# lfalive/fast-genomic-data-processing

Hardware: AMD Instinct MI355X
Metric: PairHMM GCUPS (higher is better)
Workload: dtype f32

## Files before the change

fast-genomic-data-processing_amd/csrc/pairhmm_kernels.hip.inc:

```

#include <type_traits>

namespace {

struct Job {
    uint64_t read_off;
    uint64_t hap_off;
    uint32_t R;
    uint32_t H;
    uint32_t pair;
    uint32_t pad_;
};
static_assert(sizeof(Job) == 32, "Job is 32 bytes");

struct KernelArgs {
    const Job* jobs;
    const uint32_t* job_list;
    const uint32_t* n_dyn;
    uint32_t n_static;
    uint32_t job_first;
    const uint8_t* bases;
    const uint8_t* qual;
    const uint8_t* ins;
    const uint8_t* del;
    const uint8_t* gcp;
    const uint8_t* hap_bases;
    const void* ph2pr;
    const void* mm;
    const void* ph2pr_div3;
    const void* gap_ratio;
    double* out_log10;
    uint8_t* used_f64;
    uint32_t* rerun_list;
    uint32_t* rerun_count;
    uint32_t lds_stride;
    void* strip_scratch;
    uint32_t strip_stride;
    float log10_initial_f;
    double log10_initial_d;
};

constexpr double kExactBelow = 1e-280;
constexpr int kCodeN = 4;
constexpr int kCodePad = 7;

__device__ __forceinline__ int base_code(int b) {
    int c = 0;
    c = (b == 'C') ? 1 : c;
    c = (b == 'T') ? 2 : c;
    c = (b == 'G') ? 3 : c;
    c = (b == 'N') ? kCodeN : c;
    return c;
}

__device__ __forceinline__ uint32_t base_code4(uint32_t w) {
    const uint32_t sel = (w >> 1) & 0x07070707u;
    const uint32_t code = __builtin_amdgcn_perm(0x04000000u, 0x03020100u, sel);
    const uint32_t want = __builtin_amdgcn_perm(0x4E000000u, 0x47544341u, sel);
    const uint32_t diff = want ^ w;
    const uint32_t nz = (((diff & 0x7F7F7F7Fu) + 0x7F7F7F7Fu) | diff) & 0x80808080u;
    const uint32_t ok = ((nz ^ 0x80808080u) >> 7) * 0xFFu;
    return code & ok;
}

template <int G> constexpr int lane_stride() { return G < 16 ? 16 / G : 1; }

template <int G>
__device__ __forceinline__ int dpp_shr1(int old, int v) {
    if constexpr (G == 64)
        return __builtin_amdgcn_update_dpp(old, v, 0x138 , 0xf, 0xf, false);
    else
        return __builtin_amdgcn_update_dpp(old, v, 0x110 + lane_stride<G>() , 0xf, 0xf, false);
}
template <int G>
__device__ __forceinline__ float shr1(float old, float v) {
    return __builtin_bit_cast(float, dpp_shr1<G>(__builtin_bit_cast(int, old), __builtin_bit_cast(int, v)));
}
template <int G>
__device__ __forceinline__ double shr1(double old, double v) {
    long long o = __builtin_bit_cast(long long, old), x = __builtin_bit_cast(long long, v);
    unsigned lo = (unsigned)dpp_shr1<G>((int)(unsigned)o, (int)(unsigned)x);
    unsigned hi = (unsigned)dpp_shr1<G>((int)(unsigned)(o >> 32), (int)(unsigned)(x >> 32));
    return __builtin_bit_cast(double, ((long long)hi << 32) | (long long)lo);
}

template <int G, typename T>
__device__ __forceinline__ T shr1_down(T v) {
    const int lane = (int)(threadIdx.x & 63);
    constexpr int S = lane_stride<G>();
    const int j = G < 16 ? (lane & 15) / S : lane % G;
    const int src = (j == G - 1) ? lane : lane + S;
    return __shfl(v, src, 64);
}

__device__ __forceinline__ float fma_(float a, float b, float c) { return __builtin_fmaf(a, b, c); }
__device__ __forceinline__ double fma_(double a, double b, double c) { return __builtin_fma(a, b, c); }

template <typename T> struct Prec;
template <> struct Prec<float> {
    static __device__ __forceinline__ float initial() { return 0x1p120f; }
};
template <> struct Prec<double> {
    static __device__ __forceinline__ double initial() { return 0x1p1020; }
};

#ifndef MGX_PAIRHMM_CODES
#define MGX_PAIRHMM_CODES 5
#endif
constexpr int kNumCodes = MGX_PAIRHMM_CODES;
template <int RPL> constexpr int etab_bytes_per_wave() { return ((RPL + 1) / 2) * kNumCodes * 64 * 8; }

template <typename T, int G, int RPL, bool STRIP = false, bool EXACT = false>
__device__ __forceinline__ void pairhmm_body(const KernelArgs& a, uint8_t* smem, const uint32_t block, const uint32_t n_blocks) {
    constexpr int GPW = 64 / G;
    constexpr bool kETab = (sizeof(T) == 4);
    constexpr int RP2 = (RPL + 1) / 2;
    constexpr int S = lane_stride<G>();
    const int gpb = (int)blockDim.x / G;
    const int tid = (int)threadIdx.x;
    const int lane = tid & 63;
    const int wave = tid >> 6;
    const int j = G < 16 ? (lane & 15) / S : lane % G;
    const int grp = wave * GPW + (G < 16 ? (lane >> 4) * S + (lane & 15) % S : lane / G);
    const int n_waves = (int)blockDim.x >> 6;
    uint8_t* etab = smem + (kETab ? (size_t)wave * etab_bytes_per_wave<RPL>() : 0);
    uint8_t* hapbuf = smem + (kETab ? (size_t)n_waves * etab_bytes_per_wave<RPL>() : 0) +
                      (size_t)grp * a.lds_stride;
    const T* __restrict__ ph2pr = (const T*)a.ph2pr;
    const T* __restrict__ mm = (const T*)a.mm;
    const T* __restrict__ ph2pr_div3 = (const T*)a.ph2pr_div3;
    const T* __restrict__ gap_ratio = (const T*)a.gap_ratio;
    const uint32_t n_jobs = a.n_dyn ? *a.n_dyn : a.n_static;

    for (uint32_t base = block * (uint32_t)gpb; base < n_jobs; base += n_blocks * (uint32_t)gpb) {
        const uint32_t slot = base + (uint32_t)grp;
        const bool live = slot < n_jobs;
        uint32_t job_idx = 0;
        Job job;
        job.read_off = 0; job.hap_off = 0; job.R = 0; job.H = 0; job.pair = 0; job.pad_ = 0;
        if (live) {
            job_idx = a.job_list ? a.job_list[slot] : a.job_first + slot;
            job = a.jobs[job_idx];
        }
        const int R = (int)job.R, H = (int)job.H;
        constexpr int kStripRows = G * RPL;
        const int n_strips = STRIP ? (R > kStripRows ? (R + kStripRows - 1) / kStripRows : 1) : 1;
        const int first_rows = R - (n_strips - 1) * kStripRows;

        __syncthreads();
        bool hap_n = false;
        {
            const uint8_t* hp = a.hap_bases + job.hap_off;
            const int n_words = (int)a.lds_stride >> 2;
            uint32_t* hb32 = reinterpret_cast<uint32_t*>(hapbuf);
            for (int w = j; w < n_words; w += G) {
                const int c0 = 4 * w - G;
                uint32_t packed;
                if (live && c0 >= 0 && c0 + 4 <= H) {
                    uint32_t raw;
                    __builtin_memcpy(&raw, hp + c0, 4);
                    packed = base_code4(raw);
                } else {
                    packed = 0;
#pragma unroll
                    for (int t = 0; t < 4; ++t) {
                        const int c = c0 + t;
                        const int code = (live && c >= 0 && c < H) ? base_code(hp[c]) : (kNumCodes > 4 ? kCodeN : 0);
                        packed |= (uint32_t)code << (8 * t);
                    }
                }
                if constexpr (kETab && kNumCodes == 4) {
                    const uint32_t x = packed ^ (0x01010101u * (uint32_t)kCodeN);
                    hap_n |= ((x - 0x01010101u) & ~x & 0x80808080u) != 0;
                    packed &= 0x03030303u;
                }
                hb32[w] = packed;
            }
        }
        bool group_hap_n = false;
        if constexpr (kETab && kNumCodes == 4) {
            uint64_t gmask;
            if constexpr (G == 64) gmask = ~0ull;
            else if constexpr (G == 16) gmask = 0xFFFFull << (lane & 48);
            else gmask = (uint64_t)((G == 8 ? 0x5555u : 0x1111u) << ((lane & 15) % S)) << (lane & 48);
            group_hap_n = (__ballot((int)hap_n) & gmask) != 0;
        }

        T sumM = 0, sumX = 0;
        bool zero_gap = false;
        if constexpr (STRIP) {
            for (int rr = lane; rr < R; rr += 64) zero_gap |= (a.gcp[job.read_off + (uint64_t)rr] & 127) == 0;
        }
        int nl = 0;
        T* const bnd = STRIP ? reinterpret_cast<T*>(a.strip_scratch) + (size_t)block * 6u * a.strip_stride : nullptr;
      for (int strip = 0; strip < n_strips; ++strip) {
        const int rows_here = (STRIP && strip > 0) ? kStripRows : first_rows;
        const int row_base = (STRIP && strip > 0) ? first_rows + (strip - 1) * kStripRows : 0;
        const bool last_strip = strip == n_strips - 1;
        nl = (rows_here + RPL - 1) / RPL;
        const int top_clones = nl * RPL - rows_here;
        volatile T* const bcur = STRIP ? bnd + (size_t)(strip & 1) * 3u * a.strip_stride : nullptr;
        const volatile T* const bprev = STRIP ? bnd + (size_t)((strip & 1) ^ 1) * 3u * a.strip_stride : nullptr;
        if (STRIP && strip > 0) __syncthreads();

        T k0[RPL], k1[RPL], k2[RPL], k3[RPL], k4[RPL], eM[RPL], eX[RPL];
        int rb[RPL];
        T pm[RPL], px[RPL], py[RPL];
        bool clone[RPL];
        T ratio[RPL];
        const T init_y = Prec<T>::initial() / (T)(H > 0 ? H : 1);
#pragma unroll
        for (int s = 0; s < RPL; ++s) {
            const int rho = j * RPL + s - top_clones;
            k0[s] = 0; k1[s] = 0; k2[s] = 0; k3[s] = 0; k4[s] = 0; eM[s] = 0; eX[s] = 0;
            rb[s] = 0; pm[s] = 0; px[s] = 0; py[s] = 0; clone[s] = false; ratio[s] = 0;
            if (live && j < nl) {
                if (rho < 0) {
                    clone[s] = true;
                    k3[s] = 1;
                    py[s] = init_y;
                } else {
                    const uint64_t o = job.read_off + (uint64_t)(row_base + rho);
                    const int qi = a.ins[o] & 127, qd = a.del[o] & 127, qc = a.gcp[o] & 127;
                    const int qq = a.qual[o] & 127;
                    const int mn = qi <= qd ? qi : qd, mx = qi <= qd ? qd : qi;
                    k0[s] = mm[((mx * (mx + 1)) >> 1) + mn];
                    k3[s] = ph2pr[qc];
                    k1[s] = (T)1.0 - ph2pr[qc];
                    k2[s] = ph2pr[qi];
                    k4[s] = ph2pr[qd];
                    zero_gap |= (qc == 0);
                    const T distm = ph2pr[qq];
                    eM[s] = (T)1.0 - distm;
                    const int code = base_code(a.bases[o]);
                    eX[s] = (code == kCodeN) ? eM[s] : ph2pr_div3[qq];
                    ratio[s] = gap_ratio[qc];
                    rb[s] = code;
                }
            }
        }
        if constexpr (kETab) {
            float* et = reinterpret_cast<float*>(etab) + lane * 2;
#pragma unroll
            for (int s = 0; s < RPL; ++s)
#pragma unroll
                for (int code = 0; code < kNumCodes; ++code)
                    et[((s >> 1) * kNumCodes + code) * 128 + (s & 1)] =
                        (code == rb[s] || code == kCodeN) ? eM[s] : eX[s];
        }
        __syncthreads();

        const int nsteps_g = live ? (H + nl - 1) : 0;
        int nmax = nsteps_g, nmin = live ? nsteps_g : 0x7fffffff;
        if constexpr (GPW > 1) {
#pragma unroll
            for (int off = 1; off < 64; off <<= 1) {
                if (off >= S && off < (G < 16 ? 16 : G)) continue;
                const int o1 = __shfl_xor(nmax, off, 64), o2 = __shfl_xor(nmin, off, 64);
                nmax = o1 > nmax ? o1 : nmax;
                nmin = o2 < nmin ? o2 : nmin;
            }
        }
        nmax = __builtin_amdgcn_readfirstlane(nmax);
        nmin = __builtin_amdgcn_readfirstlane(nmin);
        if (nmin > nmax) nmin = nmax;

        const uint8_t* hp_lane = hapbuf + (G - j);
        const uint8_t* et_lane = etab + lane * 8;

        auto load_e = [&](int h, T (&dst)[RPL]) {
            if constexpr (kETab) {
                const uint8_t* p = et_lane + (h << 9);
#pragma unroll
                for (int s2 = 0; s2 < RP2; ++s2) {
                    const float2 v = *reinterpret_cast<const float2*>(p + s2 * kNumCodes * 512);
                    dst[2 * s2] = v.x;
                    if (2 * s2 + 1 < RPL) dst[2 * s2 + 1] = v.y;
                }
            } else {
                const bool hN = (h == kCodeN);
#pragma unroll
                for (int s = 0; s < RPL; ++s) dst[s] = ((h == rb[s]) | hN) ? eM[s] : eX[s];
            }
        };

        const bool use_plain = EXACT || __any((int)zero_gap) != 0;

        auto sweep = [&](auto scaled_tag) {
            constexpr bool SC = decltype(scaled_tag)::value;
            T y_above = init_y;
            if constexpr (SC) {
                T g_own[RPL], g_below[RPL];
#pragma unroll
                for (int s = 0; s < RPL; ++s) g_own[s] = k1[s];
                T g_next_lane = shr1_down<G>(g_own[0]);
#pragma unroll
                for (int s = 0; s < RPL; ++s) g_below[s] = (s + 1 < RPL) ? g_own[s + 1] : g_next_lane;
                if (j == nl - 1) {
                    g_below[RPL - 1] = (T)1.0;
                    if constexpr (STRIP) { if (!last_strip) g_below[RPL - 1] = (T)1.0 - ph2pr[a.gcp[job.read_off + (uint64_t)(row_base + rows_here)] & 127]; }
                }
#pragma unroll
                for (int s = 0; s < RPL; ++s) {
                    if (clone[s]) {
                        py[s] = g_below[s] * init_y;
                    } else {
                        const T gb = g_below[s];
                        const T pMX = k2[s], pXX = k3[s], pMY = k4[s];
                        k1[s] = gb * pMX;
                        k2[s] = gb * ratio[s];
                        k3[s] = gb * pMY;
                        k4[s] = pXX;
                    }
                    if (clone[s]) { k1[s] = 0; k2[s] = 0; k3[s] = 0; k4[s] = 1; }
                }
                y_above = g_own[0] * init_y;
            }
            const T old_y = (j == 0) ? y_above : (T)0;
            T uaM = 0, uaX = 0, uaY = old_y, ubM = 0, ubX = 0, ubY = old_y;
            if constexpr (STRIP) {
                if (strip > 0) {
                    uaY = 0; ubY = 0;
                    if (j == 0 && H > 0) { ubM = bprev[0]; ubX = bprev[a.strip_stride]; ubY = bprev[2u * a.strip_stride]; }
                }
            }

            auto column = [&](const T (&ec)[RPL], T& o2M, T& o2X, T& o2Y, const T o1M, const T o1X, bool count, const int dcol) {
                T Mn[RPL], Xn[RPL], Yn[RPL];
                if constexpr (SC) {
                    Mn[0] = (fma_(o2M, k0[0], o2X) + o2Y) * ec[0];
                    Xn[0] = fma_(o1X, k2[0], o1M * k1[0]);
                    Yn[0] = fma_(py[0], k4[0], pm[0] * k3[0]);
#pragma unroll
                    for (int s = 1; s < RPL; ++s) {
                        Mn[s] = (fma_(pm[s - 1], k0[s], px[s - 1]) + py[s - 1]) * ec[s];
                        Xn[s] = fma_(Xn[s - 1], k2[s], Mn[s - 1] * k1[s]);
                        Yn[s] = fma_(py[s], k4[s], pm[s] * k3[s]);
                    }
                } else if constexpr (EXACT) {
                    Mn[0] = ((o2M * k0[0] + o2X * k1[0]) + o2Y * k1[0]) * ec[0];
                    Xn[0] = o1M * k2[0] + o1X * k3[0];
                    Yn[0] = pm[0] * k4[0] + py[0] * k3[0];
#pragma unroll
                    for (int s = 1; s < RPL; ++s) {
                        Mn[s] = ((pm[s - 1] * k0[s] + px[s - 1] * k1[s]) + py[s - 1] * k1[s]) * ec[s];
                        Xn[s] = Mn[s - 1] * k2[s] + Xn[s - 1] * k3[s];
                        Yn[s] = pm[s] * k4[s] + py[s] * k3[s];
                    }
                } else {
                    Mn[0] = fma_(o2Y, k1[0], fma_(o2X, k1[0], o2M * k0[0])) * ec[0];
                    Xn[0] = fma_(o1X, k3[0], o1M * k2[0]);
                    Yn[0] = fma_(py[0], k3[0], pm[0] * k4[0]);
#pragma unroll
                    for (int s = 1; s < RPL; ++s) {
                        Mn[s] = fma_(py[s - 1], k1[s], fma_(px[s - 1], k1[s], pm[s - 1] * k0[s])) * ec[s];
                        Xn[s] = fma_(Xn[s - 1], k3[s], Mn[s - 1] * k2[s]);
                        Yn[s] = fma_(py[s], k3[s], pm[s] * k4[s]);
                    }
                }
#pragma unroll
                for (int s = 0; s < RPL; ++s) { pm[s] = Mn[s]; px[s] = Xn[s]; py[s] = Yn[s]; }
                if (count && (!STRIP || last_strip)) { sumM += Mn[RPL - 1]; sumX += Xn[RPL - 1]; }
                o2M = shr1<G>(o2M, Mn[RPL - 1]);
                o2X = shr1<G>(o2X, Xn[RPL - 1]);
                o2Y = shr1<G>(o2Y, Yn[RPL - 1]);
                if constexpr (STRIP) {
                    if (strip > 0 && j == 0) {
                        const int c1 = dcol + 1;
                        const bool in = c1 < H;
                        o2M = in ? bprev[c1] : (T)0; o2X = in ? bprev[a.strip_stride + c1] : (T)0; o2Y = in ? bprev[2u * a.strip_stride + c1] : (T)0;
                    }
                    if (!last_strip && j == nl - 1) {
                        const int c = dcol - j;
                        if (c >= 0 && c < H) { bcur[c] = Mn[RPL - 1]; bcur[a.strip_stride + c] = Xn[RPL - 1]; bcur[2u * a.strip_stride + c] = Yn[RPL - 1]; }
                    }
                }
            };

            T e[RPL];
            int d = 0;
            int h1 = hp_lane[1];
            load_e((int)hp_lane[0], e);
            for (; d + 2 <= nmin; d += 2) {
                T e1[RPL];
                load_e(h1, e1);
                const int h2 = hp_lane[d + 2], h3 = hp_lane[d + 3];
                column(e, uaM, uaX, uaY, ubM, ubX, true, d);
                load_e(h2, e);
                column(e1, ubM, ubX, ubY, uaM, uaX, true, d + 1);
                h1 = h3;
            }
            for (; d < nmax; ++d) {
                const int hn = hp_lane[d + 1];
                column(e, uaM, uaX, uaY, ubM, ubX, d < nsteps_g, d);
                T t;
                t = uaM; uaM = ubM; ubM = t;
                t = uaX; uaX = ubX; ubX = t;
                t = uaY; uaY = ubY; ubY = t;
                load_e(hn, e);
            }
        };
        if constexpr (EXACT) sweep(std::integral_constant<bool, false>{});
        else if (use_plain) sweep(std::integral_constant<bool, false>{});
        else sweep(std::integral_constant<bool, true>{});
      }

        if (live && j == nl - 1) {
            const T res = sumM + sumX;
            if constexpr (sizeof(T) == 4) {
                if (res < 1e-28f || group_hap_n) {
                    const uint32_t k = atomicAdd(a.rerun_count, 1u);
                    a.rerun_list[k] = job_idx;
                } else {
                    a.out_log10[job.pair] = (double)(log10f(res) - a.log10_initial_f);
                }
            } else {
                if (!EXACT && a.rerun_count && res < kExactBelow) {
                    const uint32_t k = atomicAdd(a.rerun_count, 1u);
                    a.rerun_list[k] = job_idx;
                } else {
                    a.out_log10[job.pair] = log10(res) - a.log10_initial_d;
                    a.used_f64[job.pair] = 1;
                }
            }
        }
    }
}

typedef float f2 __attribute__((ext_vector_type(2)));
__device__ __forceinline__ f2 pk_fma(f2 a, f2 b, f2 c) { return __builtin_elementwise_fma(a, b, c); }

constexpr int kPkCodes = 4;
constexpr int kPkRowStride = kPkCodes * 64 * 4 + 4;
template <int P> constexpr int etab_pk_bytes_per_wave() { return (2 * P * kPkRowStride + 15) & ~15; }

template <int G, int P>
__device__ __forceinline__ void pairhmm_body_pk(const KernelArgs& a, uint8_t* smem, const uint32_t block, const uint32_t n_blocks) {
    typedef float T;
    constexpr int RPL = 2 * P;
    constexpr int GPW = 64 / G;
    constexpr int S = lane_stride<G>();
    constexpr int PAD = 2 * G;
    const int gpb = (int)blockDim.x / G;
    const int tid = (int)threadIdx.x;
    const int lane = tid & 63;
    const int wave = tid >> 6;
    const int j = G < 16 ? (lane & 15) / S : lane % G;
    const int grp = wave * GPW + (G < 16 ? (lane >> 4) * S + (lane & 15) % S : lane / G);
    const int n_waves = (int)blockDim.x >> 6;
    uint8_t* etab = smem + (size_t)wave * etab_pk_bytes_per_wave<P>();
    uint8_t* hapbuf = smem + (size_t)n_waves * etab_pk_bytes_per_wave<P>() + (size_t)grp * a.lds_stride;
    const T* __restrict__ ph2pr = (const T*)a.ph2pr;
    const T* __restrict__ mm = (const T*)a.mm;
    const T* __restrict__ ph2pr_div3 = (const T*)a.ph2pr_div3;
    const T* __restrict__ gap_ratio = (const T*)a.gap_ratio;
    const uint32_t n_jobs = a.n_dyn ? *a.n_dyn : a.n_static;

    for (uint32_t base = block * (uint32_t)gpb; base < n_jobs; base += n_blocks * (uint32_t)gpb) {
        const uint32_t slot = base + (uint32_t)grp;
        const bool live = slot < n_jobs;
        uint32_t job_idx = 0;
        Job job;
        job.read_off = 0; job.hap_off = 0; job.R = 0; job.H = 0; job.pair = 0; job.pad_ = 0;
        if (live) {
            job_idx = a.job_list ? a.job_list[slot] : a.job_first + slot;
            job = a.jobs[job_idx];
        }
        const int R = (int)job.R, H = (int)job.H;

        __syncthreads();
        bool to_f64 = false;
        {
            const uint8_t* hp = a.hap_bases + job.hap_off;
            const int n_words = (int)a.lds_stride >> 2;
            uint32_t* hb32 = reinterpret_cast<uint32_t*>(hapbuf);
            for (int w = j; w < n_words; w += G) {
                const int c0 = 4 * w - PAD;
                uint32_t packed;
                if (live && c0 >= 0 && c0 + 4 <= H) {
                    uint32_t raw;
                    __builtin_memcpy(&raw, hp + c0, 4);
                    packed = base_code4(raw);
                } else {
                    packed = 0;
#pragma unroll
                    for (int t = 0; t < 4; ++t) {
                        const int c = c0 + t;
                        const int code = (live && c >= 0 && c < H) ? base_code(hp[c]) : 0;
                        packed |= (uint32_t)code << (8 * t);
                    }
                }
                const uint32_t x = packed ^ (0x01010101u * (uint32_t)kCodeN);
                to_f64 |= ((x - 0x01010101u) & ~x & 0x80808080u) != 0;
                hb32[w] = packed & 0x03030303u;
            }
        }

        const int nh = (R + P - 1) / P;
        const int top_clones = nh * P - R;
        const int qf = nh - 1;
        const T init_y = Prec<T>::initial() / (T)(H > 0 ? H : 1);

        T g_own[RPL];
#pragma unroll
        for (int t = 0; t < RPL; ++t) {
            const int rho = j * RPL + t - top_clones;
            const int q = 2 * j + (t >= P ? 1 : 0);
            g_own[t] = 0;
            if (live && q < nh && rho >= 0) {
                const int qc = a.gcp[job.read_off + (uint64_t)rho] & 127;
                g_own[t] = (T)1.0 - ph2pr[qc];
                to_f64 |= (qc == 0);
            }
        }
        const T g_next_lane = shr1_down<G>(g_own[0]);
        f2 K0[P], K1[P], K2[P], K3[P], K4[P], pm[P], px[P], py[P];
        {
            float* et = reinterpret_cast<float*>(etab) + lane;
#pragma unroll
            for (int t = 0; t < RPL; ++t) {
                const int rho = j * RPL + t - top_clones;
                const int q = 2 * j + (t >= P ? 1 : 0);
                T gb = (t + 1 < RPL) ? g_own[t + 1] : g_next_lane;
                if (j == (qf >> 1) && t == ((qf & 1) ? RPL - 1 : P - 1)) gb = (T)1.0;
                T c0 = 0, cA = 0, cB = 0, cC = 0, cD = 0, y0 = 0, eM = 0, eX = 0;
                int rb = 0;
                if (live && q < nh) {
                    if (rho < 0) {
                        cD = 1; y0 = gb * init_y;
                    } else {
                        const uint64_t o = job.read_off + (uint64_t)rho;
                        const int qi = a.ins[o] & 127, qd = a.del[o] & 127, qc = a.gcp[o] & 127;
                        const int qq = a.qual[o] & 127;
                        const int mn = qi <= qd ? qi : qd, mx = qi <= qd ? qd : qi;
                        c0 = mm[((mx * (mx + 1)) >> 1) + mn];
                        cA = gb * ph2pr[qi];
                        cB = gb * gap_ratio[qc];
                        cC = gb * ph2pr[qd];
                        cD = ph2pr[qc];
                        eM = (T)1.0 - ph2pr[qq];
                        rb = base_code(a.bases[o]);
                        eX = (rb == kCodeN) ? eM : ph2pr_div3[qq];
                    }
                }
#pragma unroll
                for (int code = 0; code < kPkCodes; ++code)
                    et[t * (kPkRowStride / 4) + code * 64] = (code == rb) ? eM : eX;
                const int k = t % P;
                if (t < P) { K0[k].x = c0; K1[k].x = cA; K2[k].x = cB; K3[k].x = cC; K4[k].x = cD; py[k].x = y0; }
                else       { K0[k].y = c0; K1[k].y = cA; K2[k].y = cB; K3[k].y = cC; K4[k].y = cD; py[k].y = y0; }
            }
        }
#pragma unroll
        for (int k = 0; k < P; ++k) { pm[k] = f2{0, 0}; px[k] = f2{0, 0}; }
        const T y_above = g_own[0] * init_y;
        const T py_mid = py[P - 1].x;
        __syncthreads();

        const int nsteps_g = live ? (H + nh - 1) : 0;
        int nmax = nsteps_g, nmin = live ? nsteps_g : 0x7fffffff;
        if constexpr (GPW > 1) {
#pragma unroll
            for (int off = 1; off < 64; off <<= 1) {
                if (off >= S && off < (G < 16 ? 16 : G)) continue;
                const int o1 = __shfl_xor(nmax, off, 64), o2 = __shfl_xor(nmin, off, 64);
                nmax = o1 > nmax ? o1 : nmax;
                nmin = o2 < nmin ? o2 : nmin;
            }
        }
        nmax = __builtin_amdgcn_readfirstlane(nmax);
        nmin = __builtin_amdgcn_readfirstlane(nmin);
        if (nmin > nmax) nmin = nmax;

        const uint8_t* hp_lane = hapbuf + (PAD - 2 * j);
        const uint8_t* et_lane = etab + lane * 4;
        uint64_t gmask;
        if constexpr (G == 64) gmask = ~0ull;
        else if constexpr (G == 16) gmask = 0xFFFFull << (lane & 48);
        else gmask = (uint64_t)((G == 8 ? 0x5555u : 0x1111u) << ((lane & 15) % S)) << (lane & 48);
        const bool group_to_f64 = (__ballot((int)to_f64) & gmask) != 0;

        f2 sumM = {0, 0}, sumX = {0, 0};

        {
            const T old_y = (j == 0) ? y_above : (T)0;
            f2 uaM = {0, 0}, uaX = {0, 0}, uaY = {old_y, py_mid}, ubM = {0, 0}, ubX = {0, 0}, ubY = {old_y, py_mid};

            auto column = [&](const f2 (&ec)[P], f2& o2M, f2& o2X, f2& o2Y, const f2 o1M, const f2 o1X, bool count) {
                f2 Mn[P], Xn[P], Yn[P];
                Mn[0] = (pk_fma(o2M, K0[0], o2X) + o2Y) * ec[0];
                Xn[0] = pk_fma(o1X, K2[0], o1M * K1[0]);
                Yn[0] = pk_fma(py[0], K4[0], pm[0] * K3[0]);
#pragma unroll
                for (int k = 1; k < P; ++k) {
                    Mn[k] = (pk_fma(pm[k - 1], K0[k], px[k - 1]) + py[k - 1]) * ec[k];
                    Xn[k] = pk_fma(Xn[k - 1], K2[k], Mn[k - 1] * K1[k]);
                    Yn[k] = pk_fma(py[k], K4[k], pm[k] * K3[k]);
                }
#pragma unroll
                for (int k = 0; k < P; ++k) { pm[k] = Mn[k]; px[k] = Xn[k]; py[k] = Yn[k]; }
                if (count) { sumM += Mn[P - 1]; sumX += Xn[P - 1]; }
                o2M.x = shr1<G>(o2M.x, Mn[P - 1].y); o2M.y = Mn[P - 1].x;
                o2X.x = shr1<G>(o2X.x, Xn[P - 1].y); o2X.y = Xn[P - 1].x;
                o2Y.x = shr1<G>(o2Y.x, Yn[P - 1].y); o2Y.y = Yn[P - 1].x;
            };
            auto load_e = [&](int h, int hprev, f2 (&dst)[P]) {
                const uint8_t* pc = et_lane + (h << 8);
                const uint8_t* pp = et_lane + (hprev << 8) + P * kPkRowStride;
#pragma unroll
                for (int k = 0; k < P; ++k) {
                    dst[k].x = *reinterpret_cast<const float*>(pc + k * kPkRowStride);
                    dst[k].y = *reinterpret_cast<const float*>(pp + k * kPkRowStride);
                }
            };

            f2 e[P];
            int d = 0;
            int h0 = hp_lane[0], h1 = hp_lane[1];
            load_e(h0, (int)hp_lane[-1], e);
            for (; d + 2 <= nmin; d += 2) {
                f2 e1[P];
                load_e(h1, h0, e1);
                const int h2 = hp_lane[d + 2], h3 = hp_lane[d + 3];
                __builtin_amdgcn_sched_barrier(0);
                column(e, uaM, uaX, uaY, ubM, ubX, true);
                __builtin_amdgcn_sched_barrier(0);
                load_e(h2, h1, e);
                __builtin_amdgcn_sched_barrier(0);
                column(e1, ubM, ubX, ubY, uaM, uaX, true);
                __builtin_amdgcn_sched_barrier(0);
                h0 = h2; h1 = h3;
            }
            for (; d < nmax; ++d) {
                const int hn = hp_lane[d + 1];
                column(e, uaM, uaX, uaY, ubM, ubX, d < nsteps_g);
                f2 t;
                t = uaM; uaM = ubM; ubM = t;
                t = uaX; uaX = ubX; ubX = t;
                t = uaY; uaY = ubY; ubY = t;
                load_e(hn, h0, e);
                h0 = hn;
            }
        }

        if (live && j == (qf >> 1)) {
            const T res = (qf & 1) ? (sumM.y + sumX.y) : (sumM.x + sumX.x);
            if (group_to_f64 || res < 1e-28f) {
                const uint32_t k = atomicAdd(a.rerun_count, 1u);
                a.rerun_list[k] = job_idx;
            } else {
                a.out_log10[job.pair] = (double)(log10f(res) - a.log10_initial_f);
            }
        }
    }
}

#ifndef MGX_HMM_PK_MINWAVES
#define MGX_HMM_PK_MINWAVES 4
#endif
template <int G, int P>
__global__ __launch_bounds__(256, P == 4 ? MGX_HMM_PK_MINWAVES : 1) void pairhmm_fwd_pk(KernelArgs a) {
    extern __shared__ __attribute__((aligned(16))) uint8_t smem[];
    pairhmm_body_pk<G, P>(a, smem, blockIdx.x, gridDim.x);
}

template <typename T, int G, int RPL>
#ifndef MGX_HMM_MINWAVES_8
#define MGX_HMM_MINWAVES_8 4
#endif
__global__ __launch_bounds__(256, (sizeof(T) == 4 && RPL == 7) ? MGX_HMM_MINWAVES_8 : 1) void pairhmm_fwd(KernelArgs a) {
    extern __shared__ __attribute__((aligned(16))) uint8_t smem[];
    pairhmm_body<T, G, RPL>(a, smem, blockIdx.x, gridDim.x);
}

constexpr int kStripG = 64, kStripRPL = 16;
template <typename T>
__global__ __launch_bounds__(64) void pairhmm_fwd_strip(KernelArgs a) {
    extern __shared__ __attribute__((aligned(16))) uint8_t smem[];
    pairhmm_body<T, kStripG, kStripRPL, true>(a, smem, blockIdx.x, gridDim.x);
}
__global__ __launch_bounds__(64) void pairhmm_fwd_exact(KernelArgs a) {
    extern __shared__ __attribute__((aligned(16))) uint8_t smem[];
    pairhmm_body<double, kStripG, kStripRPL, true, true>(a, smem, blockIdx.x, gridDim.x);
}

constexpr int kMultiBins = 16;
struct MultiArgs {
    KernelArgs a;
    uint32_t n_bins;
    uint32_t block_first[kMultiBins + 1];
    uint32_t job_first[kMultiBins], job_count[kMultiBins], lds_stride[kMultiBins];
    uint8_t G[kMultiBins], RPL[kMultiBins];
};

template <int GSET>
__device__ __forceinline__ void pairhmm_multi_body(const MultiArgs& m, uint8_t* smem) {
    uint32_t k = 0;
    while (k + 1 < m.n_bins && blockIdx.x >= m.block_first[k + 1]) ++k;
    KernelArgs a = m.a;
    a.job_first = m.job_first[k]; a.n_static = m.job_count[k]; a.lds_stride = m.lds_stride[k];
    const uint32_t blk = blockIdx.x - m.block_first[k], nblk = m.block_first[k + 1] - m.block_first[k];
    const int code = (int)m.G[k] * 16 + (int)m.RPL[k];
#define MGX_MCASE(g, r) case (g) * 16 + (r): pairhmm_body<float, g, r>(a, smem, blk, nblk); break;
    if constexpr (GSET == 0) {
        switch (code) {
            MGX_MCASE(16, 1) MGX_MCASE(16, 2) MGX_MCASE(16, 3) MGX_MCASE(16, 4) MGX_MCASE(16, 5) MGX_MCASE(16, 6) MGX_MCASE(16, 7) MGX_MCASE(16, 8)
            default: break;
        }
    } else {
        switch (code) {
            MGX_MCASE(8, 1) MGX_MCASE(8, 2) MGX_MCASE(8, 3) MGX_MCASE(8, 4) MGX_MCASE(8, 5) MGX_MCASE(8, 6) MGX_MCASE(8, 7) MGX_MCASE(8, 8)
            MGX_MCASE(4, 1) MGX_MCASE(4, 2) MGX_MCASE(4, 3) MGX_MCASE(4, 4) MGX_MCASE(4, 5) MGX_MCASE(4, 6) MGX_MCASE(4, 7) MGX_MCASE(4, 8)
            default: break;
        }
    }
#undef MGX_MCASE
}

template <int GSET>
__global__ __launch_bounds__(256) void pairhmm_fwd_multi(MultiArgs m) {
    extern __shared__ __attribute__((aligned(16))) uint8_t smem[];
    pairhmm_multi_body<GSET>(m, smem);
}
template <int GSET>
__global__ __launch_bounds__(256) __attribute__((amdgpu_waves_per_eu(4, 4))) void pairhmm_fwd_multi_occ4(MultiArgs m) {
    extern __shared__ __attribute__((aligned(16))) uint8_t smem[];
    pairhmm_multi_body<GSET>(m, smem);
}

struct SeqRef {
    uint64_t off;
    uint32_t len;
    uint32_t id;
};
__global__ __launch_bounds__(256) void pairhmm_make_jobs(const SeqRef* __restrict__ reads, const SeqRef* __restrict__ haps,
                                                         uint32_t n_haps, uint32_t n_jobs, Job* __restrict__ jobs) {
    const uint32_t q = blockIdx.x * 256 + threadIdx.x;
    if (q >= n_jobs) return;
    const SeqRef r = reads[q / n_haps], h = haps[q % n_haps];
    Job j;
    j.read_off = r.off; j.hap_off = h.off; j.R = r.len; j.H = h.len; j.pair = r.id * n_haps + h.id; j.pad_ = 0;
    jobs[q] = j;
}

struct RegionRef {
    uint32_t hap_begin;
    uint32_t n_haps;
    uint32_t read_base;
    uint32_t out_base;
};
__global__ __launch_bounds__(256) void pairhmm_make_jobs_multi(const SeqRef* __restrict__ reads, const uint32_t* __restrict__ read_region,
                                                               const uint32_t* __restrict__ job_prefix, uint32_t n_reads,
                                                               const RegionRef* __restrict__ regions, const SeqRef* __restrict__ haps,
                                                               uint32_t n_jobs, Job* __restrict__ jobs) {
    const uint32_t q = blockIdx.x * 256 + threadIdx.x;
    if (q >= n_jobs) return;
    uint32_t lo = 0, hi = n_reads;
    while (hi - lo > 1) { const uint32_t m = lo + (hi - lo) / 2; if (job_prefix[m] <= q) lo = m; else hi = m; }
    const SeqRef r = reads[lo];
    const RegionRef g = regions[read_region[lo]];
    const SeqRef h = haps[g.hap_begin + (q - job_prefix[lo])];
    Job j;
    j.read_off = r.off; j.hap_off = h.off; j.R = r.len; j.H = h.len;
    j.pair = g.out_base + (r.id - g.read_base) * g.n_haps + h.id; j.pad_ = 0;
    jobs[q] = j;
}

struct ReadModel {
    uint8_t pcr_cache[21];
    int rate_factor;
    int bq_threshold;
    int constant_gcp;
};

__device__ __forceinline__ int n_repetitions(const uint8_t* s, int unit_off, int unit_len, int test_off, int test_len, bool leading) {
    if (test_len == 0) return 0;
    const int diff = test_len - unit_len;
    int n = 0;
    if (leading) {
        for (int st = 0; st <= diff; st += unit_len) {
            bool eq = true;
            for (int i = 0; i < unit_len; ++i) eq &= s[st + test_off + i] == s[unit_off + i];
            if (!eq) return n;
            ++n;
        }
    } else {
        for (int st = diff; st >= 0; st -= unit_len) {
            bool eq = true;
            for (int i = 0; i < unit_len; ++i) eq &= s[st + test_off + i] == s[unit_off + i];
            if (!eq) return n;
            ++n;
        }
    }
    return n;
}
__device__ int tandem_repeat_units(const uint8_t* b, int length, int offset) {
    int maxBW = 0, bw_off = offset, bw_len = 1;
    for (int str = 1; str <= 8; ++str) {
        if (offset + 1 - str < 0) break;
        maxBW = n_repetitions(b, offset - str + 1, str, 0, offset + 1, false);
        if (maxBW > 1) { bw_off = offset - str + 1; bw_len = str; break; }
    }
    int maxRL = maxBW;
    if (offset < length - 1) {
        int maxFW = 0, fw_len = 1;
        const int fw_off = offset + 1;
        for (int str = 1; str <= 8; ++str) {
            if (offset + str + 1 > length) break;
            maxFW = n_repetitions(b, offset + 1, str, offset + 1, length - offset - 1, true);
            if (maxFW > 1) { fw_len = str; break; }
        }
        bool same = fw_len == bw_len;
        if (same) for (int i = 0; i < fw_len; ++i) same &= b[fw_off + i] == b[bw_off + i];
        if (!same) maxBW = n_repetitions(b, fw_off, fw_len, 0, offset + 1, false);
        maxRL = maxFW + maxBW;
    }
    return maxRL > 20 ? 20 : maxRL;
}

__global__ __launch_bounds__(128) void pairhmm_read_model(const SeqRef* __restrict__ reads, const uint8_t* __restrict__ bases,
                                                          uint8_t* qual, uint8_t* ins, uint8_t* del, uint8_t* gcp,
                                                          const uint8_t* __restrict__ mapq, ReadModel m) {
    __shared__ uint8_t sb[1024 + 16];
    const SeqRef r = reads[blockIdx.x];
    const int len = (int)r.len;
    const bool in_lds = len <= 1024;
    if (in_lds) for (int i = threadIdx.x; i < len; i += blockDim.x) sb[i] = bases[r.off + i];
    __syncthreads();
    const uint8_t* sbp = in_lds ? sb : bases + r.off;
    const int mq = mapq[r.id];
    for (int i = threadIdx.x; i < len; i += blockDim.x) {
        int qi = ins[r.off + i], qd = del[r.off + i];
        if (m.rate_factor > 0 && i < len - 1) {
            const int c = m.pcr_cache[tandem_repeat_units(sbp, len, i)];
            qi = c < qi ? c : qi; qd = c < qd ? c : qd;
        }
        int q = qual[r.off + i];
        q = mq < q ? mq : q;
        qual[r.off + i] = (uint8_t)(q < m.bq_threshold ? 6 : q);
        ins[r.off + i] = (uint8_t)(qi < 6 ? 6 : qi);
        del[r.off + i] = (uint8_t)(qd < 6 ? 6 : qd);
        if (m.constant_gcp >= 0) gcp[r.off + i] = (uint8_t)m.constant_gcp;
    }
}

__global__ __launch_bounds__(256) void pairhmm_normalize_filter(double* __restrict__ out, const uint64_t* __restrict__ read_len,
                                                                uint32_t n_reads, uint32_t n_haps, double log10_rate,
                                                                double max_error_per_base, uint8_t* __restrict__ keep) {
    const uint32_t r = blockIdx.x * 4 + (threadIdx.x >> 6);
    const int lane = threadIdx.x & 63;
    if (r >= n_reads) return;
    double* row = out + (size_t)r * n_haps;
    double best = -__builtin_inf();
    for (uint32_t h = lane; h < n_haps; h += 64) best = fmax(best, row[h]);
#pragma unroll
    for (int off = 32; off > 0; off >>= 1) best = fmax(best, __shfl_xor(best, off, 64));
    if (!__builtin_isinf(log10_rate) && n_haps > 1) {
        const double cap = best + log10_rate;
        for (uint32_t h = lane; h < n_haps; h += 64) if (row[h] < cap) row[h] = cap;
    }
    if (lane == 0) {
        const double max_err = fmin(2.0, ceil((double)read_len[r] * max_error_per_base));
        keep[r] = !(best < max_err * -4.0);
    }
}

__global__ __launch_bounds__(256) void pairhmm_normalize_filter_rows(double* __restrict__ out, const uint64_t* __restrict__ read_len,
                                                                     const uint32_t* __restrict__ row_off, const uint32_t* __restrict__ row_nh,
                                                                     uint32_t n_reads, double log10_rate, double max_error_per_base,
                                                                     uint8_t* __restrict__ keep) {
    const uint32_t r = blockIdx.x * 4 + (threadIdx.x >> 6);
    const int lane = threadIdx.x & 63;
    if (r >= n_reads) return;
    const uint32_t n_haps = row_nh[r];
    double* row = out + row_off[r];
    double best = -__builtin_inf();
    for (uint32_t h = lane; h < n_haps; h += 64) best = fmax(best, row[h]);
#pragma unroll
    for (int off = 32; off > 0; off >>= 1) best = fmax(best, __shfl_xor(best, off, 64));
    if (!__builtin_isinf(log10_rate) && n_haps > 1) {
        const double cap = best + log10_rate;
        for (uint32_t h = lane; h < n_haps; h += 64) if (row[h] < cap) row[h] = cap;
    }
    if (lane == 0) {
        const double max_err = fmin(2.0, ceil((double)read_len[r] * max_error_per_base));
        keep[r] = !(best < max_err * -4.0);
    }
}

using KernelFn = void (*)(KernelArgs);

inline KernelFn pick_kernel_pk(int G, int P) {
#define MGX_CASE(g, p) if (G == g && P == p) return pairhmm_fwd_pk<g, p>;
    MGX_CASE(4, 1) MGX_CASE(4, 2) MGX_CASE(4, 3) MGX_CASE(4, 4)
    MGX_CASE(8, 1) MGX_CASE(8, 2) MGX_CASE(8, 3) MGX_CASE(8, 4)
    MGX_CASE(16, 1) MGX_CASE(16, 2) MGX_CASE(16, 3) MGX_CASE(16, 4)
#undef MGX_CASE
    return nullptr;
}

template <typename T>
KernelFn pick_kernel(int G, int RPL) {
#define MGX_CASE(g, r) if (G == g && RPL == r) return pairhmm_fwd<T, g, r>;
    MGX_CASE(4, 1) MGX_CASE(4, 2) MGX_CASE(4, 3) MGX_CASE(4, 4) MGX_CASE(4, 5) MGX_CASE(4, 6) MGX_CASE(4, 7) MGX_CASE(4, 8)
    MGX_CASE(8, 1) MGX_CASE(8, 2) MGX_CASE(8, 3) MGX_CASE(8, 4) MGX_CASE(8, 5) MGX_CASE(8, 6) MGX_CASE(8, 7) MGX_CASE(8, 8)
    MGX_CASE(16, 1) MGX_CASE(16, 2) MGX_CASE(16, 3) MGX_CASE(16, 4)
    MGX_CASE(16, 5) MGX_CASE(16, 6) MGX_CASE(16, 7) MGX_CASE(16, 8)
    if constexpr (sizeof(T) == 4) { MGX_CASE(16, 9) MGX_CASE(16, 10) MGX_CASE(16, 11) MGX_CASE(16, 12) }
    if constexpr (sizeof(T) == 8) { MGX_CASE(64, 3) }
    MGX_CASE(64, 4) MGX_CASE(64, 5) MGX_CASE(64, 6) MGX_CASE(64, 7) MGX_CASE(64, 8)
    MGX_CASE(64, 9) MGX_CASE(64, 10) MGX_CASE(64, 11) MGX_CASE(64, 12)
    MGX_CASE(64, 13) MGX_CASE(64, 14) MGX_CASE(64, 15) MGX_CASE(64, 16)
#undef MGX_CASE
    return nullptr;
}

}
```

Baseline: 6021.

## Rescale Y-state recurrence to six-op form folding gap factor into M update

Adds a 'six-op' scaled variant of the f32 PairHMM recurrence. The Y-state scaling factor moves from the Y update into the M update, so Y needs one fused multiply-add instead of a multiply plus an FMA. The M update absorbs the factor into its existing add via an FMA. The k3 coefficient is re-derived from the own-row gap probability times the deletion probability of the row above, which is exchanged across lanes, and the initial Y values drop the g factor. The packed kernel gets the same reformulation, and RPL=10 f32 kernels get a launch-bounds occupancy hint of 3, at some risk of numerical differences from the reassociation.

```diff
diff --git a/fast-genomic-data-processing_amd/csrc/pairhmm_kernels.hip.inc b/fast-genomic-data-processing_amd/csrc/pairhmm_kernels.hip.inc
--- a/fast-genomic-data-processing_amd/csrc/pairhmm_kernels.hip.inc
+++ b/fast-genomic-data-processing_amd/csrc/pairhmm_kernels.hip.inc
@@ -114,6 +114,7 @@
 __device__ __forceinline__ void pairhmm_body(const KernelArgs& a, uint8_t* smem, const uint32_t block, const uint32_t n_blocks) {
     constexpr int GPW = 64 / G;
     constexpr bool kETab = (sizeof(T) == 4);
+    constexpr bool kSix = (sizeof(T) == 4) && !EXACT;
     constexpr int RP2 = (RPL + 1) / 2;
     constexpr int S = lane_stride<G>();
     const int gpb = (int)blockDim.x / G;
@@ -285,11 +286,14 @@
         };
 
         const bool use_plain = EXACT || __any((int)zero_gap) != 0;
-
-        auto sweep = [&](auto scaled_tag) {
-            constexpr bool SC = decltype(scaled_tag)::value;
+        constexpr int kPlain = 0, kScaled = 1, kSixOp = 2;
+
+        auto sweep = [&](auto form_tag) {
+            constexpr int FORM = decltype(form_tag)::value;
+            constexpr bool SC = FORM == kScaled;
+            constexpr bool SIX = FORM == kSixOp;
             T y_above = init_y;
-            if constexpr (SC) {
+            if constexpr (SC || SIX) {
                 T g_own[RPL], g_below[RPL];
 #pragma unroll
                 for (int s = 0; s < RPL; ++s) g_own[s] = k1[s];
@@ -300,21 +304,35 @@
                     g_below[RPL - 1] = (T)1.0;
                     if constexpr (STRIP) { if (!last_strip) g_below[RPL - 1] = (T)1.0 - ph2pr[a.gcp[job.read_off + (uint64_t)(row_base + rows_here)] & 127]; }
                 }
+                T my_above[RPL];
+                if constexpr (SIX) {
+                    T my_own[RPL];
+#pragma unroll
+                    for (int s = 0; s < RPL; ++s) my_own[s] = clone[s] ? (T)1.0 : k4[s];
+                    T my_top = (T)1.0;
+                    if constexpr (STRIP) {
+                        if (strip > 0) my_top = ph2pr[a.del[job.read_off + (uint64_t)(row_base - 1)] & 127];
+                    }
+                    my_above[0] = shr1<G>(my_top, my_own[RPL - 1]);
+#pragma unroll
+                    for (int s = 1; s < RPL; ++s) my_above[s] = my_own[s - 1];
+                }
 #pragma unroll
                 for (int s = 0; s < RPL; ++s) {
                     if (clone[s]) {
-                        py[s] = g_below[s] * init_y;
+                        py[s] = SIX ? init_y : g_below[s] * init_y;
                     } else {
                         const T gb = g_below[s];
                         const T pMX = k2[s], pXX = k3[s], pMY = k4[s];
                         k1[s] = gb * pMX;
                         k2[s] = gb * ratio[s];
-                        k3[s] = gb * pMY;
+                        if constexpr (SIX) k3[s] = g_own[s] * my_above[s];
+                        else k3[s] = gb * pMY;
                         k4[s] = pXX;
                     }
                     if (clone[s]) { k1[s] = 0; k2[s] = 0; k3[s] = 0; k4[s] = 1; }
                 }
-                y_above = g_own[0] * init_y;
+                y_above = SIX ? init_y : g_own[0] * init_y;
             }
             const T old_y = (j == 0) ? y_above : (T)0;
             T uaM = 0, uaX = 0, uaY = old_y, ubM = 0, ubX = 0, ubY = old_y;
@@ -327,7 +345,17 @@
 
             auto column = [&](const T (&ec)[RPL], T& o2M, T& o2X, T& o2Y, const T o1M, const T o1X, bool count, const int dcol) {
                 T Mn[RPL], Xn[RPL], Yn[RPL];
-                if constexpr (SC) {
+                if constexpr (SIX) {
+                    Mn[0] = fma_(k3[0], o2Y, fma_(o2M, k0[0], o2X)) * ec[0];
+                    Xn[0] = fma_(o1X, k2[0], o1M * k1[0]);
+                    Yn[0] = fma_(py[0], k4[0], pm[0]);
+#pragma unroll
+                    for (int s = 1; s < RPL; ++s) {
+                        Mn[s] = fma_(k3[s], py[s - 1], fma_(pm[s - 1], k0[s], px[s - 1])) * ec[s];
+                        Xn[s] = fma_(Xn[s - 1], k2[s], Mn[s - 1] * k1[s]);
+                        Yn[s] = fma_(py[s], k4[s], pm[s]);
+                    }
+                } else if constexpr (SC) {
                     Mn[0] = (fma_(o2M, k0[0], o2X) + o2Y) * ec[0];
                     Xn[0] = fma_(o1X, k2[0], o1M * k1[0]);
                     Yn[0] = fma_(py[0], k4[0], pm[0] * k3[0]);
@@ -400,9 +428,10 @@
                 load_e(hn, e);
             }
         };
-        if constexpr (EXACT) sweep(std::integral_constant<bool, false>{});
-        else if (use_plain) sweep(std::integral_constant<bool, false>{});
-        else sweep(std::integral_constant<bool, true>{});
+        if constexpr (EXACT) sweep(std::integral_constant<int, kPlain>{});
+        else if (use_plain) sweep(std::integral_constant<int, kPlain>{});
+        else if constexpr (kSix) sweep(std::integral_constant<int, kSixOp>{});
+        else sweep(std::integral_constant<int, kScaled>{});
       }
 
         if (live && j == nl - 1) {
@@ -501,19 +530,24 @@
         const int qf = nh - 1;
         const T init_y = Prec<T>::initial() / (T)(H > 0 ? H : 1);
 
-        T g_own[RPL];
+        T g_own[RPL], my_own[RPL];
 #pragma unroll
         for (int t = 0; t < RPL; ++t) {
             const int rho = j * RPL + t - top_clones;
             const int q = 2 * j + (t >= P ? 1 : 0);
             g_own[t] = 0;
+            my_own[t] = 0;
             if (live && q < nh && rho >= 0) {
                 const int qc = a.gcp[job.read_off + (uint64_t)rho] & 127;
                 g_own[t] = (T)1.0 - ph2pr[qc];
+                my_own[t] = ph2pr[a.del[job.read_off + (uint64_t)rho] & 127];
                 to_f64 |= (qc == 0);
+            } else if (live && q < nh) {
+                my_own[t] = 1;
             }
         }
         const T g_next_lane = shr1_down<G>(g_own[0]);
+        const T my_prev_lane = shr1<G>((T)1.0, my_own[RPL - 1]);
         f2 K0[P], K1[P], K2[P], K3[P], K4[P], pm[P], px[P], py[P];
         {
             float* et = reinterpret_cast<float*>(etab) + lane;
@@ -527,7 +561,7 @@
                 int rb = 0;
                 if (live && q < nh) {
                     if (rho < 0) {
-                        cD = 1; y0 = gb * init_y;
+                        cD = 1; y0 = init_y;
                     } else {
                         const uint64_t o = job.read_off + (uint64_t)rho;
                         const int qi = a.ins[o] & 127, qd = a.del[o] & 127, qc = a.gcp[o] & 127;
@@ -536,7 +570,7 @@
                         c0 = mm[((mx * (mx + 1)) >> 1) + mn];
                         cA = gb * ph2pr[qi];
                         cB = gb * gap_ratio[qc];
-                        cC = gb * ph2pr[qd];
+                        cC = g_own[t] * (t > 0 ? my_own[t - 1] : my_prev_lane);
                         cD = ph2pr[qc];
                         eM = (T)1.0 - ph2pr[qq];
                         rb = base_code(a.bases[o]);
@@ -553,7 +587,7 @@
         }
 #pragma unroll
         for (int k = 0; k < P; ++k) { pm[k] = f2{0, 0}; px[k] = f2{0, 0}; }
-        const T y_above = g_own[0] * init_y;
+        const T y_above = init_y;
         const T py_mid = py[P - 1].x;
         __syncthreads();
 
@@ -588,14 +622,14 @@
 
             auto column = [&](const f2 (&ec)[P], f2& o2M, f2& o2X, f2& o2Y, const f2 o1M, const f2 o1X, bool count) {
                 f2 Mn[P], Xn[P], Yn[P];
-                Mn[0] = (pk_fma(o2M, K0[0], o2X) + o2Y) * ec[0];
+                Mn[0] = pk_fma(K3[0], o2Y, pk_fma(o2M, K0[0], o2X)) * ec[0];
                 Xn[0] = pk_fma(o1X, K2[0], o1M * K1[0]);
-                Yn[0] = pk_fma(py[0], K4[0], pm[0] * K3[0]);
+                Yn[0] = pk_fma(py[0], K4[0], pm[0]);
 #pragma unroll
                 for (int k = 1; k < P; ++k) {
-                    Mn[k] = (pk_fma(pm[k - 1], K0[k], px[k - 1]) + py[k - 1]) * ec[k];
+                    Mn[k] = pk_fma(K3[k], py[k - 1], pk_fma(pm[k - 1], K0[k], px[k - 1])) * ec[k];
                     Xn[k] = pk_fma(Xn[k - 1], K2[k], Mn[k - 1] * K1[k]);
-                    Yn[k] = pk_fma(py[k], K4[k], pm[k] * K3[k]);
+                    Yn[k] = pk_fma(py[k], K4[k], pm[k]);
                 }
 #pragma unroll
                 for (int k = 0; k < P; ++k) { pm[k] = Mn[k]; px[k] = Xn[k]; py[k] = Yn[k]; }
@@ -668,7 +702,7 @@
 #ifndef MGX_HMM_MINWAVES_8
 #define MGX_HMM_MINWAVES_8 4
 #endif
-__global__ __launch_bounds__(256, (sizeof(T) == 4 && RPL == 7) ? MGX_HMM_MINWAVES_8 : 1) void pairhmm_fwd(KernelArgs a) {
+__global__ __launch_bounds__(256, (sizeof(T) == 4 && RPL == 7) ? MGX_HMM_MINWAVES_8 : (sizeof(T) == 4 && RPL == 10) ? 3 : 1) void pairhmm_fwd(KernelArgs a) {
     extern __shared__ __attribute__((aligned(16))) uint8_t smem[];
     pairhmm_body<T, G, RPL>(a, smem, blockIdx.x, gridDim.x);
 }
```

After: 6194 (median of 6 runs). 1.03x the previous value.
